# tatsuki1107/Relevance-FactorizationMachine

Measured on AMD Instinct MI355X. Metric: training examples/sec (FM, k=32), higher is better.
Workload: dtype f64; 1 GPU; kuairec_big: synthetic KuaiRec-big-shaped log 7176x10728 + 110 side-feature columns, n_features=18014, 15 nnz/row, N_train=1000000, FM k=32, IPS, lr=9e-06, batch_size=65536 rows per GPU (global 65536), step = gather+forward+residual+gradients+SGD update; row-id lists precomputed; batch_size_per_gpu=65536, global_batch=65536, parallelism=single

## Files before the change

### relevance_factorizationmachine_amd/csrc/rfm_device_utils.hpp

```cpp
#pragma once

#include <hip/hip_runtime.h>

namespace rfm {

constexpr double kLogitClip = 700.0;

template <int CTRL>
__device__ inline double dpp_move(double v) {
  int lo = __double2loint(v), hi = __double2hiint(v);
  lo = __builtin_amdgcn_update_dpp(0, lo, CTRL, 0xF, 0xF, false);
  hi = __builtin_amdgcn_update_dpp(0, hi, CTRL, 0xF, 0xF, false);
  return __hiloint2double(hi, lo);
}

template <int LPR>
__device__ inline double group_sum(double v) {
  if (LPR >= 2) v += dpp_move<0xB1>(v);
  if (LPR >= 4) v += dpp_move<0x4E>(v);
  if (LPR >= 8) v += dpp_move<0x141>(v);
  if (LPR >= 16) v += dpp_move<0x140>(v);
  if (LPR >= 32) v += __shfl_xor(v, 16, 64);
  if (LPR >= 64) v += __shfl_xor(v, 32, 64);
  return v;
}

__device__ inline double sigmoid_clipped(double z) {
  z = z != z ? z : fmin(fmax(z, -kLogitClip), kLogitClip);
  return 1.0 / (1.0 + exp(-z));
}

template <int VEC>
struct Pack;
template <>
struct Pack<1> {
  double v[1];
  __device__ inline void load(const double* p) { v[0] = *p; }
  __device__ inline void store(double* p) const { *p = v[0]; }
  __device__ inline void store_through(double* p) const { store(p); }
};
template <>
struct Pack<2> {
  double v[2];
  __device__ inline void load(const double* p) {
    const double2 t = *reinterpret_cast<const double2*>(p);
    v[0] = t.x;
    v[1] = t.y;
  }
  __device__ inline void store(double* p) const {
    *reinterpret_cast<double2*>(p) = make_double2(v[0], v[1]);
  }
  __device__ inline void store_through(double* p) const {
    typedef double f64x2 __attribute__((ext_vector_type(2)));
    const f64x2 t = {v[0], v[1]};
    asm volatile("global_store_dwordx4 %0, %1, off sc1\n\ts_nop 1" ::"v"(p), "v"(t) : "memory");
  }
};

}
```

### relevance_factorizationmachine_amd/csrc/rfm_fm.hip

```cpp
#include <algorithm>
#include <atomic>
#include <cmath>
#include <cstdlib>
#include <memory>
#include <numeric>
#include <string>
#include <thread>

#include "rfm_common.h"
#include "rfm_fm_kernels.hpp"
#include "rfm_fm_plan.h"
#include "rfm_fm_rows.hpp"
#include "rfm_fm_sliced.hpp"

static_assert(RFM_MAX_FACTORS <= 1024, "fm_finalize_kernel's LDS totals hold 1024+2 values");

namespace rfm {

struct FwdGeom {
  int block, grid;
};
constexpr int kSmallBlock = 256;

inline FwdGeom forward_geom(const rfm_ctx* ctx, int64_t n_rows, const Shape& s, bool records) {
  constexpr int per_cu = kBigBlock >= 1024 ? 1 : 2;
  FwdGeom g;
  const int64_t rows_big = int64_t(kBigBlock / s.lpr) * (records ? rows_in_flight(s.nc) : rows_in_flight_plain(s.nc));
  const int64_t blocks_big = (n_rows + rows_big - 1) / rows_big;
  if (blocks_big * 2 >= int64_t(ctx->n_cu) * per_cu) {
    g.block = kBigBlock;
    g.grid = capped_grid(ctx, n_rows, rows_big, per_cu, 1);
  } else {
    g.block = kSmallBlock;
    g.grid = capped_grid(ctx, n_rows, kSmallBlock / s.lpr, 8, 1);
  }
  g.grid = std::min(g.grid, 2048);
  return g;
}

int forward_grid(const rfm_ctx* ctx, int64_t rows, int n_factors) {
  return forward_geom(ctx, rows, shape_for(n_factors), true).grid;
}

bool forward_many_rows(const rfm_ctx* ctx, int64_t rows, int n_factors) {
  return forward_geom(ctx, rows, shape_for(n_factors), true).block == kBigBlock;
}

template <int L, int Vv, int N, int BLOCK, int R, bool REC, bool ELL, bool DET, bool SEG = false, bool XTRA = false>
void launch_forward_as(rfm_ctx* ctx, const FwdArgs& a, const FwdGeom& geom, size_t lds) {
  const auto kern = &fm_forward_kernel<L, Vv, N, BLOCK, R, REC, ELL, DET, SEG, XTRA>;
  static LdsLimits allowed;
  allow_dynamic_lds(ctx, reinterpret_cast<const void*>(kern), lds, allowed);
  hipLaunchKernelGGL(kern, dim3(geom.grid), dim3(BLOCK), lds, ctx->stream, a);
}

template <int L, int Vv, int N>
void launch_forward_shape(rfm_ctx* ctx, const FwdArgs& a, const FwdGeom& geom, size_t lds,
                          bool recs, bool fixed) {
  constexpr int R = rows_in_flight(N);
  if (geom.block == kBigBlock) {
    if (!recs) return launch_forward_as<L, Vv, N, kBigBlock, rows_in_flight_plain(N), false, false, false>(ctx, a, geom, lds);
    if constexpr (hot_fixed_order(L, N, kBigBlock, R)) {
      if (fixed) {
        if (a.ell) return launch_forward_as<L, Vv, N, kBigBlock, R, true, true, true>(ctx, a, geom, lds);
        return launch_forward_as<L, Vv, N, kBigBlock, R, true, false, true>(ctx, a, geom, lds);
      }
    }
    RFM_REQUIRE(!fixed, "fixed-order hot sums are not built for this factor count at this batch");
    if (a.ell) return launch_forward_as<L, Vv, N, kBigBlock, R, true, true, false>(ctx, a, geom, lds);
    RFM_REQUIRE(a.ent && a.rows, "the plan holds no row records");
    return launch_forward_as<L, Vv, N, kBigBlock, R, true, false, false>(ctx, a, geom, lds);
  }
  if (!recs) return launch_forward_as<L, Vv, N, kSmallBlock, 1, false, false, false>(ctx, a, geom, lds);
  if constexpr (hot_fixed_order(L, N, kSmallBlock, 1)) {
    if (fixed) {
      if (a.ell) return launch_forward_as<L, Vv, N, kSmallBlock, 1, true, true, true>(ctx, a, geom, lds);
      return launch_forward_as<L, Vv, N, kSmallBlock, 1, true, false, true>(ctx, a, geom, lds);
    }
  }
  RFM_REQUIRE(!fixed, "fixed-order hot sums are not built for this factor count");
  if (a.n_rows_x > 0) {
    if (a.ell) return launch_forward_as<L, Vv, N, kSmallBlock, 1, true, true, false, false, true>(ctx, a, geom, lds);
    RFM_REQUIRE(a.ent && a.rows, "the plan holds no row records");
    return launch_forward_as<L, Vv, N, kSmallBlock, 1, true, false, false, false, true>(ctx, a, geom, lds);
  }
  if (a.ell) return launch_forward_as<L, Vv, N, kSmallBlock, 1, true, true, false>(ctx, a, geom, lds);
  RFM_REQUIRE(a.ent && a.rows, "the plan holds no row records");
  return launch_forward_as<L, Vv, N, kSmallBlock, 1, true, false, false>(ctx, a, geom, lds);
}

bool forward_fixed_order_ok(const rfm_ctx* ctx, int64_t max_batch, int n_factors) {
  const Shape s = shape_for(n_factors);
  if (!hot_fixed_order(s.lpr, s.nc, kSmallBlock, 1)) return false;
  return !forward_many_rows(ctx, max_batch, n_factors) ||
         hot_fixed_order(s.lpr, s.nc, kBigBlock, rows_in_flight(s.nc));
}

void launch_forward(rfm_ctx* ctx, FwdArgs a, FwdGeom geom) {
  if (a.n_rows <= 0) return;
  const Shape s = shape_for(a.k);
  const bool recs = a.ent != nullptr || a.ell != nullptr;
  const bool fixed = recs && a.hot_fixed && a.n_hot > 0;
  const size_t lds =
      forward_lds_bytes(geom.block, s.lpr, s.vec, s.nc,
                        geom.block == kBigBlock ? (recs ? rows_in_flight(s.nc) : rows_in_flight_plain(s.nc)) : 1,
                        a.n_hot, a.k, fixed);
  RFM_REQUIRE(lds <= (160u << 10), "forward kernel: %zu bytes of LDS", lds);
  RFM_REQUIRE(!fixed || a.hot_rounds >= 1, "hot_rounds unset");
#define RFM_CALL_FWD(L, Vv, N) launch_forward_shape<L, Vv, N>(ctx, a, geom, lds, recs, fixed)
  RFM_FOR_SHAPE(s, RFM_CALL_FWD);
#undef RFM_CALL_FWD
  RFM_HIP_CHECK(hipGetLastError());
}

void launch_forward(rfm_ctx* ctx, FwdArgs a) {
  if (a.n_rows <= 0) return;
  launch_forward(ctx, a, forward_geom(ctx, a.n_rows, shape_for(a.k), a.ent != nullptr || a.ell != nullptr));
}

void forward_loss(rfm_ctx* ctx, FwdArgs a, double* d_out_loss) {
  RFM_REQUIRE(a.n_rows > 0, "loss of zero rows");
  const FwdGeom geom = forward_geom(ctx, a.n_rows, shape_for(a.k), a.ent != nullptr || a.ell != nullptr);
  ctx->loss_partials.ensure(size_t(std::max(kMaxFwdGrid, ctx->n_cu * 8)) * sizeof(double));
  a.loss_partial = ctx->loss_partials.as<double>();
  launch_forward(ctx, a, geom);
  hipLaunchKernelGGL(loss_finish_kernel, dim3(1), dim3(kBlock), 0, ctx->stream,
                     ctx->loss_partials.as<double>(), geom.grid, a.n_rows, d_out_loss);
  RFM_HIP_CHECK(hipGetLastError());
}

int forward_loss_pair_deferred(rfm_ctx* ctx, FwdArgs a, double* row_a, double* row_b) {
  const Shape s = shape_for(a.k);
  const FwdGeom geom = forward_geom(ctx, a.n_rows, s, false);
  if (geom.block != kBigBlock || geom.grid > kMaxFwdGrid) return -1;
  a.loss_partial = row_a;
  a.loss_partial2 = row_b;
  const size_t lds = forward_lds_bytes(geom.block, s.lpr, s.vec, s.nc, rows_in_flight_plain(s.nc), 0, a.k, false);
#define RFM_CALL_SEG(L, Vv, N) \
  launch_forward_as<L, Vv, N, kBigBlock, rows_in_flight_plain(N), false, false, false, true>(ctx, a, geom, lds)
  RFM_FOR_SHAPE(s, RFM_CALL_SEG);
#undef RFM_CALL_SEG
  RFM_HIP_CHECK(hipGetLastError());
  return geom.grid;
}

int forward_loss_deferred(rfm_ctx* ctx, FwdArgs a, double* partial_row) {
  RFM_REQUIRE(a.n_rows > 0, "loss of zero rows");
  const FwdGeom geom = forward_geom(ctx, a.n_rows, shape_for(a.k), a.ent != nullptr || a.ell != nullptr);
  RFM_REQUIRE(geom.grid <= kMaxFwdGrid, "forward grid %d exceeds %d", geom.grid, kMaxFwdGrid);
  a.loss_partial = partial_row;
  launch_forward(ctx, a, geom);
  return geom.grid;
}

struct SlicedGeom {
  bool ok = false;
  int grid = 0, rows_per_wg = 0;
  size_t lds = 0;
};
SlicedGeom sliced_geom(const rfm_ctx* ctx, const rfm_fm_plan* plan, int64_t rows, int64_t form_rows = -1) {
  SlicedGeom g;
  if (plan->sl_ns <= 0 || env_int("RFM_SLICED_LOSS", 1) == 0) return g;
  if ((form_rows >= 0 ? form_rows : rows) < std::max(1, env_int("RFM_SLICED_MIN_ROWS", 4096))) return g;
  if (rows >= (int64_t(1) << 31) - 1) return g;
  const int xs = 8 / plan->sl_ns;
  int wps = std::max(xs, ctx->n_cu / plan->sl_ns / xs * xs);
  const int64_t min_rows = kSlWaves * 4;
  while (wps > xs && rows / wps < min_rows) wps -= xs;
  g.rows_per_wg = int(std::min<int64_t>((rows + wps - 1) / wps, INT32_MAX));
  g.lds = sliced_lds_bytes(plan->sl_n_cached, plan->sl_sw);
  if (g.lds > size_t(kSlicedLds)) return g;
  g.grid = 8 * (wps / xs);
  g.ok = true;
  return g;
}

SlicedArgs plan_sliced_args(const rfm_fm_plan* plan, const double* w0, const double* w, const double* V,
                            double* zpart) {
  SlicedArgs a{};
  a.tr_a = plan->sl_train.as<SlEnt>();
  a.pad = plan->sl_pad.as<SlEnt>();
  a.w0 = w0;
  a.w = w;
  a.V = V;
  a.k = plan->k;
  a.ns = plan->sl_ns;
  a.sw = plan->sl_sw;
  a.n_cached = plan->sl_n_cached;
  a.cached_cols = plan->sl_cols.as<int32_t>();
  a.cached_rank = plan->sl_rank.as<int32_t>();
  a.ml_log2 = plan->sl_ml_log2;
  a.zpart = zpart;
  return a;
}

void launch_sliced(rfm_ctx* ctx, const SlicedGeom& g, SlicedArgs a) {
  a.rows_per_wg = g.rows_per_wg;
  static LdsLimits allowed;
  allow_dynamic_lds(ctx, reinterpret_cast<const void*>(&fm_logit_slices_kernel), g.lds, allowed);
  hipLaunchKernelGGL(fm_logit_slices_kernel, dim3(g.grid), dim3(kSlBlock), g.lds, ctx->stream, a);
  RFM_HIP_CHECK(hipGetLastError());
}

}

using namespace rfm;

namespace {

void check_step_args(const rfm_fm_plan* plan, const void* indptr, const void* indices,
                     const void* values, const void* y, const void* p, const void* ids,
                     int64_t batch) {
  RFM_REQUIRE(plan, "null plan");
  RFM_REQUIRE(indptr && indices && values && y && p && ids, "null pointer");
  RFM_REQUIRE(batch >= 1 && batch <= plan->max_batch, "batch=%lld outside 1..max_batch=%lld",
              (long long)batch, (long long)plan->max_batch);
}

void validate_ids(rfm_ctx* ctx, rfm_fm_plan* plan, const int32_t* d_ids, int64_t batch,
                  int64_t n_iters) {
  if (env_int("RFM_CHECK_IDS", 0) == 0 || batch <= 0 || n_iters <= 0) return;
  if (!plan->ids_seen.p || plan->ids_stamp > INT32_MAX - n_iters - 2) {
    plan->ids_seen.ensure(size_t(plan->n_rows) * 4);
    plan->ids_flags.ensure(8);
    RFM_HIP_CHECK(hipMemsetAsync(plan->ids_seen.p, 0, plan->ids_seen.bytes, ctx->stream));
    plan->ids_stamp = 0;
  }
  RFM_HIP_CHECK(hipMemsetAsync(plan->ids_flags.p, 0, 8, ctx->stream));
  const int64_t total = batch * n_iters;
  const int grid = capped_grid(ctx, total, kBlock, 8, 0);
  hipLaunchKernelGGL(ids_check_kernel, dim3(grid), dim3(kBlock), 0, ctx->stream, d_ids, batch,
                     n_iters, plan->n_rows, plan->ids_seen.as<int32_t>(), plan->ids_stamp + 1,
                     plan->ids_flags.as<int32_t>());
  plan->ids_stamp += int32_t(n_iters);
  int32_t flags[2] = {0, 0};
  RFM_HIP_CHECK(hipMemcpyAsync(flags, plan->ids_flags.p, 8, hipMemcpyDeviceToHost, ctx->stream));
  RFM_HIP_CHECK(hipStreamSynchronize(ctx->stream));
  RFM_REQUIRE(!flags[0], "a row id lies outside the plan's log (0..%lld)", (long long)plan->n_rows - 1);
  RFM_REQUIRE(!flags[1], "a row id occurs twice in one batch: the ids of a step must be distinct");
}

struct XtraRows {
  const int32_t* ids;
  int64_t n;
  double* out_pred;
  const RowRec* rows_y;
  const Entry* ent_y;
  int64_t n_y;
  double* out_pred_y;
};

FwdArgs plan_fwd_args(const rfm_fm_plan* plan, const int32_t* ids, int64_t n, const double* w0,
                      const double* w, const double* V) {
  FwdArgs f{};
  f.ent = plan->ent.as<Entry>();
  f.rows = plan->rows.as<RowRec>();
  f.ell = plan->ell.as<char>();
  f.ell_stride = plan->ell_stride;
  f.ell_yp = plan->ell_yp.as<double2>();
  f.row_ids = ids;
  f.n_rows = n;
  f.w0 = w0;
  f.w = w;
  f.V = V;
  f.k = plan->k;
  return f;
}

int launch_step_forward(rfm_ctx* ctx, FwdArgs f, const XtraRows* xtra) {
  const Shape s = shape_for(f.k);
  const FwdGeom geom = forward_geom(ctx, f.n_rows, s, true);
  FwdGeom launch = geom;
  if (xtra && xtra->n > 0) {
    RFM_REQUIRE(geom.block == kSmallBlock && !(f.hot_fixed && f.n_hot > 0),
                "this step cannot score extra rows");
    const FwdGeom gx = forward_geom(ctx, xtra->n, s, true);
    RFM_REQUIRE(gx.block == kSmallBlock, "extra rows: unexpected geometry");
    f.grid_main = geom.grid;
    f.grid_x = gx.grid;
    f.row_ids_x = xtra->ids;
    f.n_rows_x = xtra->n;
    f.out_pred_x = xtra->out_pred;
    launch.grid = geom.grid + gx.grid;
    if (xtra->n_y > 0) {
      const FwdGeom gy = forward_geom(ctx, xtra->n_y, s, true);
      RFM_REQUIRE(gy.block == kSmallBlock && f.ent && f.rows, "extra log: unexpected geometry / plan form");
      f.rows_y = xtra->rows_y;
      f.ent_y = xtra->ent_y;
      f.n_rows_y = xtra->n_y;
      f.out_pred_y = xtra->out_pred_y;
      launch.grid += gy.grid;
    }
  }
  ctx->prof_mark();
  launch_forward(ctx, f, launch);
  ctx->prof_mark();
  return geom.grid;
}

template <class O>
void launch_consume(rfm_ctx* ctx, ConsArgs c, const Shape& s, const O& o) {
  const int grid = c.nb_tasks + c.n_hot + 1;
  const size_t lds = consume_lds_bytes(s.lpr, c.c.k);
  if (s.nc > 1) {
    const int n_chunks = fm_chunks(c.c.k, s.vec);
    c.n_chunks = n_chunks;
    c.xcd_chunks = n_chunks <= 8 ? 1 : 0;
    const int per_chunk = 8 / n_chunks;
    const dim3 g2 = c.xcd_chunks ? dim3(8 * ((grid + per_chunk - 1) / per_chunk)) : dim3(grid, n_chunks);
    const auto a = args_under(c, o);
    if (s.vec == 2)
      hipLaunchKernelGGL((fm_consume_kernel<64, 2, true, O>), g2, dim3(kBlock), lds, ctx->stream, a);
    else
      hipLaunchKernelGGL((fm_consume_kernel<64, 1, true, O>), g2, dim3(kBlock), lds, ctx->stream, a);
  } else {
    const auto a = args_under(c, o);
#define RFM_CALL_CONS(L, Vv, N) \
  hipLaunchKernelGGL((fm_consume_kernel<L, Vv, false, O>), dim3(grid), dim3(kBlock), lds, ctx->stream, a)
    RFM_FOR_SINGLE_CHUNK_SHAPE(s, RFM_CALL_CONS);
#undef RFM_CALL_CONS
  }
  RFM_HIP_CHECK(hipGetLastError());
}

template <class O>
void launch_finalize(rfm_ctx* ctx, const FinArgs& fa, const Shape& s, const O& o) {
  const int gpb = kBlock / s.lpr;
  const int nb_short = (fa.n_split_short + gpb - 1) / gpb;
  const int grid = nb_short + fa.n_split_long;
  const auto a = args_under(fa, o);
  if (s.nc > 1) {
    const dim3 g2(grid, fm_chunks(fa.c.k, s.vec));
    if (s.vec == 2)
      hipLaunchKernelGGL((fm_finalize_chunk_kernel<2, O>), g2, dim3(kBlock), 0, ctx->stream, a, nb_short);
    else
      hipLaunchKernelGGL((fm_finalize_chunk_kernel<1, O>), g2, dim3(kBlock), 0, ctx->stream, a, nb_short);
  } else {
#define RFM_CALL_FIN(L, Vv, N) \
  hipLaunchKernelGGL((fm_finalize_kernel<L, Vv, O>), dim3(grid), dim3(kBlock), 0, ctx->stream, a, nb_short)
    RFM_FOR_SINGLE_CHUNK_SHAPE(s, RFM_CALL_FIN);
#undef RFM_CALL_FIN
  }
  RFM_HIP_CHECK(hipGetLastError());
}

template <class O>
void launch_updates(rfm_ctx* ctx, const rfm_fm_plan* plan, const ConsArgs& c, const Shape& s, const O& o) {
  launch_consume(ctx, c, s, o);
  ctx->prof_mark();
  if (plan->n_split_short + plan->n_split_long > 0) {
    FinArgs fa{};
    fa.c = c.c;
    fa.split = plan->split.as<SplitCol>();
    fa.n_split_short = plan->n_split_short;
    fa.n_split_long = plan->n_split_long;
    launch_finalize(ctx, fa, s, o);
  }
  ctx->prof_mark();
}

void enqueue_step(rfm_ctx* ctx, rfm_fm_plan* plan, const int32_t* d_row_ids, int64_t batch, double* d_w0,
                  double* d_w, double* d_V, double lr, double* d_grad, int32_t* d_touch = nullptr,
                  int32_t touch_id = 0, const XtraRows* xtra = nullptr) {
  const int k = plan->k;
  const Shape s = shape_for(k);
  FwdArgs f = plan_fwd_args(plan, d_row_ids, batch, d_w0, d_w, d_V);
  f.out_Q = plan->Q.as<double>();
  f.slot_mark = plan->slot_t.as<SlotMark>();
  const bool chunked = s.nc > 1;
  const int64_t parity = chunked ? ((plan->step + 1) & 1) : 0;
  unsigned long long* bits = plan->slot_bits.as<unsigned long long>() + parity * plan->bits_words;
  unsigned long long* bits_other =
      plan->slot_bits.as<unsigned long long>() + (1 - parity) * plan->bits_words;
  f.slot_bits = bits;
  f.n_hot = plan->n_hot;
  f.hot_rounds = plan->hot_rounds;
  f.hot_fixed = plan->hot_fixed ? 1 : 0;
  f.hot_slab = plan->hot_slab.as<double>();
  f.err_partial = plan->err_partial.as<double>();
  const int n_slabs = launch_step_forward(ctx, f, xtra);

  if (d_grad && !d_touch) {
    const size_t bytes = (size_t(plan->n_features) * (k + 1) + 1) * sizeof(double);
    RFM_HIP_CHECK(hipMemsetAsync(d_grad, 0, bytes, ctx->stream));
  }
  ColArgs col{};
  col.V = d_V;
  col.w = d_w;
  col.k = k;
  col.n = plan->n_features;
  col.lr = lr;
  col.grad = d_grad;
  col.touch = d_touch;
  col.touch_id = touch_id;
  col.parts = plan->parts.as<double>();
  col.stamp = double(++plan->step);
  ConsArgs c{};
  c.c = col;
  c.tasks = plan->tasks.as<TaskRec>();
  c.task_words = plan->task_words;
  c.pool = consume_pools(plan->task_words, plan->max_batch, plan->n_rows) ? 1 : 0;
  c.slot_bits = bits;
  c.slot_bits_other = bits_other;
  c.slot_mark = plan->slot_t.as<SlotMark>();
  c.slots = plan->slots.as<SlotRec>();
// ... 665 lines not shown
```

### relevance_factorizationmachine_amd/csrc/rfm_fm_kernels.hpp

```cpp
#pragma once

#include <hip/amd_detail/amd_hip_unsafe_atomics.h>
#include <hip/hip_runtime.h>

#include <cstdint>
#include <type_traits>

#include "rfm_device_utils.hpp"
#include "rfm_fm_records.h"
#include "rfm_rule.hpp"

namespace rfm {

template <int BLOCK>
__device__ inline double block_sum(double v, double* lds) {
  const int tid = threadIdx.x;
  __syncthreads();
  lds[tid] = v;
  __syncthreads();
#pragma unroll
  for (int s = BLOCK / 2; s > 0; s >>= 1) {
    if (tid < s) lds[tid] += lds[tid + s];
    __syncthreads();
  }
  return lds[0];
}

__device__ inline double logloss_term(double y, double p, double pred, double eps) {
  const double r = y / p;
  return r * log(pred + eps) + (1.0 - r) * log(1.0 - pred + eps);
}

constexpr int kBigBlock = 1024;
constexpr int kBigWaves = 4;
constexpr int kFwdRows = 2;

constexpr int kBigUnroll = 3;
constexpr int kSmallUnroll = 8;
constexpr int kSmallWideUnroll = 2;

constexpr int rows_in_flight(int nc) { return nc == 1 ? kFwdRows : 1; }
constexpr int kFwdRowsPlain = kFwdRows;
constexpr int kPlainUnroll = kBigUnroll;
constexpr int rows_in_flight_plain(int nc) { return nc == 1 ? kFwdRowsPlain : 1; }

constexpr bool hot_fixed_order(int lpr, int nc, int block, int rows) {
  return nc == 1 && (block / lpr) * rows <= 128;
}
constexpr int kTileRanks = 16;
constexpr bool hot_tile(int lpr, int vec, int nc) { return lpr == 16 && vec == 2 && nc == 1; }
constexpr int kHotUnroll = 2;
constexpr int kHotPosPad = 4;
inline size_t forward_lds_bytes(int block, int lpr, int vec, int nc, int rows, int n_hot, int k,
                                bool fixed_order) {
  size_t bytes = size_t(block) * 8 + (size_t(block) * rows + size_t(block / lpr)) * sizeof(Entry) +
                 size_t(n_hot) * size_t(k + 2) * 8;
  if (block == kBigBlock && n_hot == 0) bytes += 2 * size_t(block / lpr) * rows * 24;
  if (!fixed_order && n_hot > 0 && hot_tile(lpr, vec, nc))
    bytes += size_t(block / lpr) * rows * kTileRanks * 8;
  if (fixed_order && n_hot > 0 && hot_fixed_order(lpr, nc, block, rows)) {
    const size_t rt = size_t(block / lpr) * rows;
    bytes += rt * size_t(lpr * vec) * 8;
    if (rt / 32 > 1) bytes += size_t(block / lpr) * size_t(k + 2) * 8;
    bytes += ((size_t(n_hot) * ((rt + 31) / 32) + 1) & ~size_t(1)) * 4;
    bytes += (size_t(n_hot) * (rt + kHotPosPad) + 7) / 8 * 8;
  }
  return bytes;
}

struct FwdArgs {
  const Entry* ent;
  const RowRec* rows;
  const char* ell;
  int64_t ell_stride;
  const double2* ell_yp;
  const int64_t* indptr;
  const int32_t* indices;
  const double* values;
  const double* y;
  const double* pscore;
  const int32_t* row_ids;
  int64_t n_rows;
  int64_t n_rows_a;
  const int64_t* indptr2;
  const int32_t* indices2;
  const double* values2;
  const double* y2;
  const double* pscore2;
  double* loss_partial2;
  const double* w0;
  const double* w;
  const double* V;
  int32_t k;
  double* out_pred;
  double* out_err;
  double* out_Q;
  SlotMark* slot_mark;
  unsigned long long* slot_bits;
  int32_t n_hot;
  int32_t hot_rounds;
  int32_t hot_fixed;
  double* hot_slab;
  double* err_partial;
  double* loss_partial;
  double eps;
  int32_t grid_main;
  const int32_t* row_ids_x;
  int64_t n_rows_x;
  double* out_pred_x;
  int32_t grid_x;
  const RowRec* rows_y;
  const Entry* ent_y;
  int64_t n_rows_y;
  double* out_pred_y;
};

struct HotEnt {
  int32_t off;
  int32_t pad;
  double coef;
};
static_assert(sizeof(HotEnt) == sizeof(Entry), "HotEnt replaces an Entry in place");

template <int LPR, int VEC, int NC, int BLOCK, int R, bool REC, bool ELL = false, bool DET = false,
          bool SEG = false, bool XTRA = false>
__global__ __launch_bounds__(BLOCK, (BLOCK == kBigBlock ? kBigWaves : 1)) void fm_forward_kernel(
    FwdArgs a) {
  constexpr int GPB = BLOCK / LPR;
  unsigned bx = blockIdx.x, gx = gridDim.x;
  if constexpr (XTRA && REC) {
    if (int(blockIdx.x) >= a.grid_main) {
      const bool second = int(blockIdx.x) >= a.grid_main + a.grid_x;
      bx = blockIdx.x - a.grid_main - (second ? a.grid_x : 0);
      gx = second ? gridDim.x - a.grid_main - a.grid_x : a.grid_x;
      a.row_ids = second ? nullptr : a.row_ids_x;
      a.n_rows = second ? a.n_rows_y : a.n_rows_x;
      if (second) {
        a.rows = a.rows_y;
        a.ent = a.ent_y;
      }
      a.n_hot = 0;
      a.slot_mark = nullptr;
      a.slot_bits = nullptr;
      a.out_Q = nullptr;
      a.out_err = nullptr;
      a.err_partial = nullptr;
      a.loss_partial = nullptr;
      a.out_pred = second ? a.out_pred_y : a.out_pred_x;
    } else {
      gx = a.grid_main;
    }
  }
  constexpr bool seg = SEG && !REC;
  extern __shared__ double dyn_lds[];
  const int tid = threadIdx.x;
  const int l = tid % LPR;
  const int g = tid / LPR;
  const int k = a.k;
  const int hot_w = k + 2;
  const int H = a.n_hot;
  double* red = dyn_lds;
  Entry* ebuf = reinterpret_cast<Entry*>(dyn_lds + BLOCK) + g * (R * LPR + 1);
  double* hot = dyn_lds + BLOCK + 2 * (BLOCK * R + GPB);
  constexpr bool FIX = DET && REC && hot_fixed_order(LPR, NC, BLOCK, R);
  constexpr int RT = GPB * R;
  constexpr int KS = LPR * VEC;
  constexpr int NW = (RT + 31) / 32;
  constexpr int NCELL = RT / 32 > 1 ? RT / 32 : 1;
  constexpr int NHV = NCELL > 1 ? GPB / NCELL : 0;
  constexpr int PS = RT + kHotPosPad;
  double* Qs = hot + H * hot_w;
  constexpr bool TILE = REC && !DET && hot_tile(LPR, VEC, NC);
  double* part = Qs + RT * KS;
  unsigned int* hbits = reinterpret_cast<unsigned int*>(part + (NCELL > 1 ? GPB * hot_w : 0));
  uint8_t* hpos = reinterpret_cast<uint8_t*>(hbits + ((H * NW + 1) & ~1));
  const double w0 = a.w0[0];
  const int64_t last_row = a.n_rows - 1;
  double loss_acc = 0.0, loss_acc2 = 0.0, err_acc = 0.0;
  const bool stage_loss = BLOCK == kBigBlock && a.loss_partial != nullptr && H == 0;
  double* lstage = hot;
  int trip = 0;
  int fo[NC];
  bool fok[NC];
#pragma unroll
  for (int c = 0; c < NC; ++c) {
    const int f = (c * LPR + l) * VEC;
    fok[c] = f < k;
    fo[c] = fok[c] ? f : 0;
  }

  if (H > 0) {
    for (int i = tid; i < H * hot_w; i += BLOCK) hot[i] = 0.0;
    if (FIX)
      for (int i = tid; i < H * NW; i += BLOCK) hbits[i] = 0u;
    __syncthreads();
  }
  for (int64_t base = int64_t(bx) * (GPB * R); base < a.n_rows;
       base += int64_t(gx) * (GPB * R)) {
    int64_t t[R];
    int32_t r[R];
    using EntryOff = typename std::conditional<REC, int32_t, int64_t>::type;
    EntryOff p0[R];
    int len[R];
    double yy[R], pp[R];
    bool valid[R];
#pragma unroll
    for (int i = 0; i < R; ++i) {
      t[i] = base + i * GPB + g;
      valid[i] = t[i] <= last_row;
      r[i] = int32_t(valid[i] ? t[i] : last_row);
    }
    bool sb[R];
#pragma unroll
    for (int i = 0; i < R; ++i) sb[i] = seg && (valid[i] ? t[i] : last_row) >= a.n_rows_a;
    if (a.row_ids) {
#pragma unroll
      for (int i = 0; i < R; ++i) r[i] = a.row_ids[sb[i] ? 0 : r[i]];
    }
    if constexpr (seg) {
#pragma unroll
      for (int i = 0; i < R; ++i)
        if (sb[i]) r[i] = int32_t((valid[i] ? t[i] : last_row) - a.n_rows_a);
    }
    int32_t nxt[R];
    const int64_t nbase = base + int64_t(gx) * (GPB * R);
    constexpr bool ell = REC && ELL;
    const bool warm = ell && BLOCK == kBigBlock && a.row_ids && nbase < a.n_rows;
    int32_t* parked = reinterpret_cast<int32_t*>(red);
    if (warm) {
#pragma unroll
      for (int i = 0; i < R; ++i) {
        const int64_t nt = nbase + i * GPB + g;
        nxt[i] = a.row_ids[nt <= last_row ? nt : last_row];
      }
    }
    Entry e0[R];
    if (ell) {
#pragma unroll
      for (int i = 0; i < R; ++i) {
        e0[i] = reinterpret_cast<const Entry*>(a.ell + int64_t(r[i]) * a.ell_stride)[l];
        const double2 yp = a.ell_yp[r[i]];
        yy[i] = yp.x;
        pp[i] = yp.y;
        p0[i] = 0;
      }
      constexpr int GPW = kWave / LPR;
#pragma unroll
      for (int i = 0; i < R; ++i) {
        unsigned long long live = __ballot(e0[i].slot != kNilSlot);
        if (GPW > 1) live = (live >> ((g % GPW) * LPR)) & ((1ull << (LPR % 64)) - 1ull);
        len[i] = valid[i] ? __popcll(live) : 0;
      }
    }
#pragma unroll
    for (int i = 0; i < R; ++i) {
      if (ell) {
      } else if (REC) {
        const RowRec rec = a.rows[r[i]];
        p0[i] = EntryOff(rec.begin);
        len[i] = valid[i] ? int(rec.len) : 0;
        yy[i] = rec.y;
        pp[i] = rec.p;
      } else {
        const int64_t* ip = sb[i] ? a.indptr2 : a.indptr;
        const int64_t b0 = ip[r[i]], b1 = ip[r[i] + 1];
        p0[i] = EntryOff(b0);
        len[i] = valid[i] ? int(b1 - b0) : 0;
        yy[i] = 0.0;
        pp[i] = 1.0;
      }
    }
    if (!REC && a.y) {
#pragma unroll
      for (int i = 0; i < R; ++i) {
        yy[i] = (sb[i] ? a.y2 : a.y)[r[i]];
        pp[i] = (sb[i] ? a.pscore2 : a.pscore)[r[i]];
      }
    }
    int maxlen = len[0];
#pragma unroll
    for (int i = 1; i < R; ++i) maxlen = max(maxlen, len[i]);
    if (warm) {
#pragma unroll
      for (int i = 0; i < R; ++i)
        if (l == 0) parked[i * GPB + g] = nxt[i];
    }

    double q[R][NC][VEC];
    double s2[R], lin[R], err[R];
#pragma unroll
    for (int i = 0; i < R; ++i) {
      s2[i] = 0.0;
      lin[i] = 0.0;
      err[i] = 0.0;
#pragma unroll
      for (int c = 0; c < NC; ++c)
#pragma unroll
        for (int v = 0; v < VEC; ++v) q[i][c][v] = 0.0;
    }

    for (int pb = 0; pb < maxlen; pb += LPR) {
      Entry e[R];
#pragma unroll
      for (int i = 0; i < R; ++i) {
        const int my = pb + l;
        const EntryOff at = len[i] > 0 ? p0[i] + min(my, len[i] - 1) : 0;
        if (ell) {
          e[i] = e0[i];
        } else if (REC) {
          e[i] = a.ent[at];
        } else {
          e[i].col = (sb[i] ? a.indices2 : a.indices)[at];
          e[i].slot = 0;
          e[i].x = (sb[i] ? a.values2 : a.values)[at];
        }
        if (my >= len[i]) {
          e[i].slot = 0;
          e[i].x = 0.0;
        }
      }
#pragma unroll
      for (int i = 0; i < R; ++i) {
        lin[i] += a.w[e[i].col] * e[i].x;
        ebuf[i * LPR + l] = e[i];
      }
      const int cnt = (maxlen - pb) < LPR ? (maxlen - pb) : LPR;
#pragma unroll(BLOCK == kBigBlock || NC > 1 ? (NC == 1 && !DET && (ELL || !REC) ? (REC ? kBigUnroll : kPlainUnroll) : (BLOCK == kBigBlock || NC > 4 ? 2 : kSmallWideUnroll)) : kSmallUnroll)
      for (int j = 0; j < cnt; ++j) {
        Entry ej[R];
        Pack<VEC> pv[R][NC];
#pragma unroll
        for (int i = 0; i < R; ++i) {
          ej[i] = ebuf[i * LPR + j];
          const double* vrow = a.V + int64_t(ej[i].col) * k;
#pragma unroll
          for (int c = 0; c < NC; ++c) pv[i][c].load(vrow + fo[c]);
        }
#pragma unroll
        for (int i = 0; i < R; ++i) {
#pragma unroll
          for (int c = 0; c < NC; ++c) {
            const double xm = fok[c] ? ej[i].x : 0.0;
#pragma unroll
            for (int v = 0; v < VEC; ++v) {
              const double vx = pv[i][c].v[v] * xm;
              q[i][c][v] += vx;
              s2[i] += vx * vx;
            }
          }
        }
      }
    }

    if (warm) {
#pragma unroll
      for (int i = 0; i < R; ++i) nxt[i] = parked[i * GPB + g];
    }
#pragma unroll
    for (int i = 0; i < R; ++i) asm volatile("" ::"v"(yy[i]), "v"(pp[i]));
#pragma unroll
    for (int i = 0; i < R; ++i) {
      if (len[i] == 0) {
        s2[i] = 0.0;
        lin[i] = 0.0;
#pragma unroll
        for (int c = 0; c < NC; ++c)
#pragma unroll
          for (int v = 0; v < VEC; ++v) q[i][c][v] = 0.0;
      }
      double pair = -s2[i];
#pragma unroll
      for (int c = 0; c < NC; ++c)
#pragma unroll
        for (int v = 0; v < VEC; ++v) pair += q[i][c][v] * q[i][c][v];
      pair = group_sum<LPR>(pair);
      const double linsum = group_sum<LPR>(lin[i]);
      const double pred = sigmoid_clipped(w0 + linsum + 0.5 * pair);
      err[i] = valid[i] ? yy[i] / pp[i] - pred : 0.0;
      if (valid[i]) {
        if (a.out_Q) {
          const uint32_t qoff = uint32_t(t[i]) * uint32_t(k);
#pragma unroll
          for (int c = 0; c < NC; ++c) {
            if (fok[c]) {
              Pack<VEC> pq;
#pragma unroll
              for (int v = 0; v < VEC; ++v) pq.v[v] = q[i][c][v];
              if (REC)
                pq.store_through(a.out_Q + (qoff + uint32_t(fo[c])));
              else
                pq.store(a.out_Q + (qoff + uint32_t(fo[c])));
            }
          }
        }
        if (l == 0) {
          if (a.out_pred) a.out_pred[t[i]] = pred;
          if (a.out_err) a.out_err[t[i]] = err[i];
          if (a.loss_partial) {
            if (stage_loss) {
              double* st = lstage + ((trip & 1) * RT + i * GPB + g) * 3;
              st[0] = pred;
              st[1] = yy[i];
              st[2] = pp[i];
            } else if (sb[i]) {
              loss_acc2 += logloss_term(yy[i], pp[i], pred, a.eps);
            } else {
              loss_acc += logloss_term(yy[i], pp[i], pred, a.eps);
            }
          }
          err_acc += err[i];
        }
      } else if (stage_loss && l == 0) {
        lstage[((trip & 1) * RT + i * GPB + g) * 3] = -1.0;
      }
    }
    if (stage_loss) {
      __syncthreads();
      if (tid < RT) {
        const double* st = lstage + ((trip & 1) * RT + tid) * 3;
        if (!(st[0] < 0.0)) {
          const double term = logloss_term(st[1], st[2], st[0], a.eps);
          if (seg && base + tid >= a.n_rows_a)
            loss_acc2 += term;
          else
            loss_acc += term;
        }
      }
    }
    ++trip;

// ... 1157 lines not shown
```

Before: 1.443 billion examples/s.

## Add 8-lanes-per-row forward kernel for k<=32 ELL training path

Adds a specialised forward kernel that assigns 8 lanes per row, each lane holding two entries and two 2-wide factor chunks, instead of the default lane mapping. It fuses the Q output, slot marking, hot-feature accumulation (including an MFMA tile for the first 16 hot ranks) and error partial sums, and dispatches to it when the ELL layout with 16 entries per row and k in (16,32] is in use. The goal is to process twice as many rows per wave and cut lane idling for k=32. The cost is a large new code path with tricky LDS aliasing and a reordered floating-point accumulation.

```diff
diff --git a/relevance_factorizationmachine_amd/csrc/rfm_device_utils.hpp b/relevance_factorizationmachine_amd/csrc/rfm_device_utils.hpp
--- a/relevance_factorizationmachine_amd/csrc/rfm_device_utils.hpp
+++ b/relevance_factorizationmachine_amd/csrc/rfm_device_utils.hpp
@@ -24,6 +24,8 @@
   if (LPR >= 64) v += __shfl_xor(v, 32, 64);
   return v;
 }
+
+__device__ inline double dpp_across_8(double v) { return dpp_move<0x128>(v); }
 
 __device__ inline double sigmoid_clipped(double z) {
   z = z != z ? z : fmin(fmax(z, -kLogitClip), kLogitClip);
diff --git a/relevance_factorizationmachine_amd/csrc/rfm_fm.hip b/relevance_factorizationmachine_amd/csrc/rfm_fm.hip
--- a/relevance_factorizationmachine_amd/csrc/rfm_fm.hip
+++ b/relevance_factorizationmachine_amd/csrc/rfm_fm.hip
@@ -101,6 +101,14 @@
   const Shape s = shape_for(a.k);
   const bool recs = a.ent != nullptr || a.ell != nullptr;
   const bool fixed = recs && a.hot_fixed && a.n_hot > 0;
+  if (geom.block == kBigBlock && a.ell && !fixed && forward_lanes8(a.k) && a.out_Q && a.slot_mark &&
+      !a.loss_partial && a.n_rows_x == 0 && a.ell_stride == int64_t(16 * sizeof(Entry))) {
+    const size_t lds8 = forward_lanes8_lds_bytes(geom.block, a.n_hot, a.k);
+    RFM_REQUIRE(lds8 <= (160u << 10), "forward kernel: %zu bytes of LDS", lds8);
+    launch_forward_as<8, 2, 2, kBigBlock, 1, true, true, false>(ctx, a, geom, lds8);
+    RFM_HIP_CHECK(hipGetLastError());
+    return;
+  }
   const size_t lds =
       forward_lds_bytes(geom.block, s.lpr, s.vec, s.nc,
                         geom.block == kBigBlock ? (recs ? rows_in_flight(s.nc) : rows_in_flight_plain(s.nc)) : 1,
diff --git a/relevance_factorizationmachine_amd/csrc/rfm_fm_kernels.hpp b/relevance_factorizationmachine_amd/csrc/rfm_fm_kernels.hpp
--- a/relevance_factorizationmachine_amd/csrc/rfm_fm_kernels.hpp
+++ b/relevance_factorizationmachine_amd/csrc/rfm_fm_kernels.hpp
@@ -49,6 +49,7 @@
 }
 constexpr int kTileRanks = 16;
 constexpr bool hot_tile(int lpr, int vec, int nc) { return lpr == 16 && vec == 2 && nc == 1; }
+constexpr bool forward_lanes8(int k) { return k > 16 && k <= 32 && k % 4 == 0; }
 constexpr int kHotUnroll = 2;
 constexpr int kHotPosPad = 4;
 inline size_t forward_lds_bytes(int block, int lpr, int vec, int nc, int rows, int n_hot, int k,
@@ -66,6 +67,9 @@
     bytes += (size_t(n_hot) * (rt + kHotPosPad) + 7) / 8 * 8;
   }
   return bytes;
+}
+inline size_t forward_lanes8_lds_bytes(int block, int n_hot, int k) {
+  return forward_lds_bytes(block, 16, 2, 1, kFwdRows, n_hot, k, false);
 }
 
 struct FwdArgs {
@@ -122,10 +126,261 @@
 };
 static_assert(sizeof(HotEnt) == sizeof(Entry), "HotEnt replaces an Entry in place");
 
+template <int BLOCK>
+__device__ inline void fm_forward_lanes8(const FwdArgs& a) {
+  constexpr int LPR = 8, VEC = 4, EPR = 16;
+  constexpr int GPB = BLOCK / LPR, GPW = kWave / LPR;
+  static_assert(kTileRanks == 16 && EPR == 2 * LPR, "one tile of 16 ranks; two entries per lane");
+  static_assert(GPB * (EPR + 1) <= BLOCK * kFwdRows + BLOCK / 16 + BLOCK / 16, "row buffers reach at most 1 KiB into red");
+  extern __shared__ double dyn_lds[];
+  const int tid = threadIdx.x;
+  const int l = tid % LPR;
+  const int g = tid / LPR;
+  const int k = a.k;
+  const int hot_w = k + 2;
+  const int H = a.n_hot;
+  const unsigned bx = blockIdx.x, gx = gridDim.x;
+  double* red = dyn_lds;
+  double* hot = dyn_lds + BLOCK + 2 * (BLOCK * kFwdRows + BLOCK / 16);
+  Entry* ebuf = reinterpret_cast<Entry*>(hot) - (GPB - g) * (EPR + 1);
+  const int rt = (g & 1) * (GPB / 2) + (g >> 1);
+  const double w0 = a.w0[0];
+  const int64_t last_row = a.n_rows - 1;
+  double err_acc = 0.0;
+  const int f0 = 2 * l, f1 = 16 + 2 * l;
+  const bool fok[2] = {true, f1 < k};
+  const int fo[2] = {fok[0] ? f0 : 0, fok[1] ? f1 : 0};
+
+  if (H > 0) {
+    for (int i = tid; i < H * hot_w; i += BLOCK) hot[i] = 0.0;
+    __syncthreads();
+  }
+  for (int64_t base = int64_t(bx) * GPB; base < a.n_rows; base += int64_t(gx) * GPB) {
+    const int64_t t = base + rt;
+    const bool valid = t <= last_row;
+    int32_t r = int32_t(valid ? t : last_row);
+    if (a.row_ids) r = a.row_ids[r];
+    const int64_t nbase = base + int64_t(gx) * GPB;
+    const bool warm = a.row_ids && nbase < a.n_rows;
+    int32_t nxt = 0;
+    if (warm) nxt = a.row_ids[nbase + rt <= last_row ? nbase + rt : last_row];
+    Entry e[2];
+#pragma unroll
+    for (int n = 0; n < 2; ++n) e[n] = reinterpret_cast<const Entry*>(a.ell + int64_t(r) * a.ell_stride)[2 * l + n];
+    const double2 yp = a.ell_yp[r];
+    int len = 0;
+#pragma unroll
+    for (int n = 0; n < 2; ++n) {
+      const unsigned long long live = __ballot(e[n].slot != kNilSlot);
+      len += __popc(unsigned(live >> ((g % GPW) * LPR)) & ((1u << LPR) - 1u));
+    }
+    if (!valid) len = 0;
+    double lin = 0.0;
+#pragma unroll
+    for (int n = 0; n < 2; ++n) {
+      if (2 * l + n >= len) {
+        e[n].slot = 0;
+        e[n].x = 0.0;
+      }
+      const double term = __builtin_fma(a.w[e[n].col], e[n].x, 0.0);
+      lin = n == 0 ? term : lin + term;
+      ebuf[2 * l + n] = e[n];
+    }
+
+    double q[VEC], s2[2];
+#pragma unroll
+    for (int v = 0; v < VEC; ++v) q[v] = 0.0;
+    s2[0] = s2[1] = 0.0;
+#pragma unroll(kBigUnroll)
+    for (int j = 0; j < len; ++j) {
+      const Entry ej = ebuf[j];
+      const double* vrow = a.V + int64_t(ej.col) * k;
+      Pack<2> pv[2];
+#pragma unroll
+      for (int n = 0; n < 2; ++n) pv[n].load(vrow + fo[n]);
+#pragma unroll
+      for (int n = 0; n < 2; ++n) {
+        const double xm = fok[n] ? ej.x : 0.0;
+#pragma unroll
+        for (int v = 0; v < 2; ++v) {
+          const double vx = pv[n].v[v] * xm;
+          q[2 * n + v] = __builtin_fma(pv[n].v[v], xm, q[2 * n + v]);
+          s2[n] = __builtin_fma(vx, vx, s2[n]);
+        }
+      }
+    }
+
+    asm volatile("" ::"v"(yp.x), "v"(yp.y));
+    if (len == 0) {
+      s2[0] = s2[1] = 0.0;
+      lin = 0.0;
+#pragma unroll
+      for (int v = 0; v < VEC; ++v) q[v] = 0.0;
+    }
+    double half[2];
+#pragma unroll
+    for (int n = 0; n < 2; ++n)
+      half[n] = __builtin_fma(q[2 * n + 1], q[2 * n + 1], __builtin_fma(q[2 * n], q[2 * n], -s2[n]));
+    const double pair = group_sum<LPR>(half[0]) + group_sum<LPR>(half[1]);
+    const double linsum = group_sum<LPR>(lin);
+    const double pred = sigmoid_clipped(w0 + linsum + 0.5 * pair);
+    const double err = valid ? yp.x / yp.y - pred : 0.0;
+    if (valid) {
+      if (a.out_Q) {
+#pragma unroll
+        for (int n = 0; n < 2; ++n) {
+          if (fok[n]) {
+            Pack<2> pq;
+            pq.v[0] = q[2 * n];
+            pq.v[1] = q[2 * n + 1];
+            pq.store_through(a.out_Q + (uint32_t(t) * uint32_t(k) + uint32_t(fo[n])));
+          }
+        }
+      }
+      if (l == 0) {
+        if (a.out_pred) a.out_pred[t] = pred;
+        if (a.out_err) a.out_err[t] = err;
+      }
+    }
+    {
+      const double second = dpp_across_8(err);
+      if (tid % 16 == 0) {
+        err_acc += err;
+        err_acc += second;
+      }
+    }
+
+    int32_t touched = 0;
+    if (warm)
+      touched = *reinterpret_cast<const int32_t*>(a.ell + int64_t(nxt) * a.ell_stride + 32 * l);
+    if (a.slot_mark || H > 0) {
+      Entry em[2];
+#pragma unroll
+      for (int n = 0; n < 2; ++n) em[n] = ebuf[2 * l + n];
+      if (a.slot_mark) {
+#pragma unroll
+        for (int n = 0; n < 2; ++n) {
+          if (2 * l + n < len && em[n].slot >= 0) {
+            Pack<2> pm;
+            pm.v[0] = __hiloint2double(0, int32_t(t));
+            pm.v[1] = err;
+            pm.store_through(reinterpret_cast<double*>(a.slot_mark + em[n].slot));
+            atomicOr(a.slot_bits + (em[n].slot >> 6), 1ull << (em[n].slot & 63));
+          }
+        }
+      }
+      if (H > 0) {
+        typedef double tile_acc __attribute__((ext_vector_type(4)));
+        int tid_here = tid;
+        asm volatile("" : "+v"(tid_here));
+        const int lh = tid_here % LPR, gh = tid_here / LPR, gw = gh % GPW;
+        const int l16 = tid_here % 16, slice = (tid_here % kWave) / 16;
+        const bool upper = (tid_here & LPR) != 0;
+        HotEnt* const hbuf = reinterpret_cast<HotEnt*>(ebuf);
+        double* const strip = hot + H * hot_w;
+        const bool rowok = valid && __builtin_isfinite(err);
+        double* const st = strip + gh * kTileRanks;
+        Pack<2> zero;
+        zero.v[0] = zero.v[1] = 0.0;
+        zero.store(st + 2 * lh);
+        bool won[2];
+        unsigned long long walked[2];
+#pragma unroll
+        for (int n = 0; n < 2; ++n) {
+          const bool live = 2 * l + n < len && em[n].slot < 0;
+          const int h = -1 - em[n].slot;
+          const bool tile_e = live && rowok && h < kTileRanks;
+          won[n] = live && !tile_e;
+          walked[n] = __ballot(won[n]);
+          const double coef = err * em[n].x;
+          if (live) {
+            double* const hsum = hot + (-em[n].slot * hot_w - 2);
+            unsafeAtomicAdd(hsum, coef);
+            unsafeAtomicAdd(hsum + 1, coef * em[n].x);
+          }
+          if (tile_e) st[h] = coef;
+        }
+        int wcnt = 0;
+#pragma unroll
+        for (int gq = 0; gq < GPW; ++gq)
+          wcnt = max(wcnt, __popc(unsigned(walked[0] >> (gq * LPR)) & ((1u << LPR) - 1u)) +
+                               __popc(unsigned(walked[1] >> (gq * LPR)) & ((1u << LPR) - 1u)));
+        const int rot = (gw * wcnt) / GPW;
+        {
+          const unsigned b0 = unsigned(walked[0] >> (gw * LPR)) & ((1u << LPR) - 1u);
+          const unsigned b1 = unsigned(walked[1] >> (gw * LPR)) & ((1u << LPR) - 1u);
+          const unsigned lower = (1u << lh) - 1u;
+          const int n0 = __popc(b0), nw = n0 + __popc(b1);
+#pragma unroll
+          for (int n = 0; n < 2; ++n) {
+            const int below = n == 0 ? __popc(b0 & lower) : n0 + __popc(b1 & lower);
+            const int p = won[n] ? below : nw + n * LPR + lh - below;
+            const int at = p - rot < 0 ? p - rot + wcnt : p - rot;
+            if (p < wcnt)
+              hbuf[at] = HotEnt{won[n] ? (-1 - em[n].slot) * hot_w : -1, 0, err * em[n].x};
+          }
+        }
+        const double c0 = strip[(gh & ~1) * kTileRanks + l16];
+        const double c1 = strip[(gh | 1) * kTileRanks + l16];
+#pragma unroll
+        for (int vp = 0; vp < VEC / 2; ++vp) {
+          const double even = rowok ? q[2 * vp] : 0.0, odd = rowok ? q[2 * vp + 1] : 0.0;
+          const double odd_across = dpp_across_8(odd), even_across = dpp_across_8(even);
+          const double b0 = upper ? odd_across : even;
+          const double b1 = upper ? odd : even_across;
+          tile_acc D = tile_acc{0.0, 0.0, 0.0, 0.0};
+          D = __builtin_amdgcn_mfma_f64_16x16x4f64(c0, b0, D, 0, 0, 0);
+          D = __builtin_amdgcn_mfma_f64_16x16x4f64(c1, b1, D, 0, 0, 0);
+          const int f = 16 * vp + 2 * (l16 % LPR) + (upper ? 1 : 0);
+#pragma unroll
+          for (int reg = 0; reg < 4; ++reg) {
+            const int rank = slice + 4 * reg;
+            if (rank < H && f < k) unsafeAtomicAdd(hot + rank * hot_w + f, D[reg]);
+          }
+        }
+        for (int j = 0; j < wcnt; ++j) {
+          const HotEnt eh = hbuf[j];
+          if (eh.off >= 0) {
+#pragma unroll
+            for (int n = 0; n < 2; ++n) {
+              if (fok[n]) {
+                double* hrow = hot + eh.off + fo[n];
+#pragma unroll
+                for (int v = 0; v < 2; ++v) unsafeAtomicAdd(hrow + v, eh.coef * q[2 * n + v]);
+              }
+            }
+          }
+        }
+      }
+    }
+    if (warm) asm volatile("" ::"v"(touched));
+  }
+
+  if (H > 0) {
+    __syncthreads();
+    for (int i = 2 * tid; i < H * hot_w; i += 2 * BLOCK) {
+      const int h = i / hot_w, f = i % hot_w;
+      Pack<2> ps;
+      ps.load(hot + i);
+      ps.store_through(a.hot_slab + (int64_t(h) * gx + bx) * hot_w + f);
+    }
+  }
+  if (a.err_partial) {
+    const double s = block_sum<BLOCK>(err_acc, red);
+    if (tid == 0) a.err_partial[bx] = s;
+  }
+}
+
 template <int LPR, int VEC, int NC, int BLOCK, int R, bool REC, bool ELL = false, bool DET = false,
           bool SEG = false, bool XTRA = false>
 __global__ __launch_bounds__(BLOCK, (BLOCK == kBigBlock ? kBigWaves : 1)) void fm_forward_kernel(
     FwdArgs a) {
+  if constexpr (LPR == 8 && NC == 2) {
+    static_assert(VEC == 2 && BLOCK == kBigBlock && R == 1 && REC && ELL && !DET && !SEG && !XTRA,
+                  "two chunks of 8 lanes: the 8-lane training forward only");
+    fm_forward_lanes8<BLOCK>(a);
+    return;
+  }
   constexpr int GPB = BLOCK / LPR;
   unsigned bx = blockIdx.x, gx = gridDim.x;
   if constexpr (XTRA && REC) {
```

Measured after the change: 1.520 billion examples/s, median of 6. +5.4%, better.
